# bailuding/rails

Measured on AMD Instinct MI355X. Metric: queries/sec, MoL exact top-k over N items (get_top_k_outputs: score + top-k' + id map + seen-id filter), higher is better.
Workload: dtype f32

## Files before the change

### rails_amd/csrc/mol_score_shell.h

```cpp
#pragma once
#include <hip/hip_runtime.h>
#include <stdlib.h>
#include <type_traits>

#include "mol_kernels.h"
#include "mol_layout.h"

namespace mol {

struct Fp32Unit;
struct Fp32UnitRows;

typedef float f32x16 __attribute__((ext_vector_type(16)));

template <class G, int NW>
__device__ __forceinline__ void stage_weights(const ScoreArgs& p, float* smem) {
  const int lane = threadIdx.x & 63, wave = __builtin_amdgcn_readfirstlane(threadIdx.x >> 6);
  constexpr int kPieces = G::kWpackFloats / 256;
  for (int piece = wave; piece < kPieces; piece += NW)
    __builtin_amdgcn_global_load_lds((const __attribute__((address_space(1))) void*)(p.wpack + piece * 256 + lane * 4),
                                     (__attribute__((address_space(3))) void*)(smem + piece * 256), 16, 0, 0);
  for (int i = kPieces * 256 + threadIdx.x; i < G::kWpackFloats; i += NW * 64) smem[i] = p.wpack[i];
}

template <class U, int PQ, int PX, int DD, int H, int NW, bool INDEXED = false>
__global__ __launch_bounds__(NW * 64, NW / 4) void mol_score_direct_kernel(ScoreArgs p) {
  using G = Geo<PQ, PX, DD, H>;
  MOL_RUN_IF(p.run_if);
  extern __shared__ __attribute__((aligned(16))) float smem[];
  U::template stage<G, NW>(p, smem);
  __syncthreads();

  const int lane = threadIdx.x & 63;
  const int wave = __builtin_amdgcn_readfirstlane(threadIdx.x >> 6);
  const int hi = lane >> 5, x = lane & 31;
  const int inner = p.per_row ? (int)p.n_tiles : p.n_groups;
  const int64_t n_units = p.per_row ? (int64_t)p.B * p.n_tiles : p.n_tiles * p.n_groups;
  const int64_t stride = (int64_t)gridDim.x * NW;
  const int64_t rounds = n_units / stride;
  const int64_t bx = (gridDim.x % 8 == 0) ? (int64_t)(blockIdx.x % 8) * (gridDim.x / 8) + blockIdx.x / 8 : (int64_t)blockIdx.x;
  for (int64_t it = 0; it <= rounds; ++it) {
    const int64_t u = it < rounds ? it * stride + bx * NW + wave
                                  : rounds * stride + (int64_t)wave * gridDim.x + bx;
    if (u >= n_units) break;
    const int64_t outer = u / inner;
    const int innr = (int)(u - outer * inner);
    const int64_t tile = p.per_row ? innr : outer;
    const int row = p.per_row ? (int)outer : -1;
    const int g = p.per_row ? row / G::QT : innr;
    const int64_t tile_addr = p.per_row ? (int64_t)row * p.n_tiles + tile : tile;
    const float4* tEx = reinterpret_cast<const float4*>(p.ipack + tile_addr * (int64_t)G::kTileFloats);
    if constexpr (INDEXED) {
      int col = (int)tile * kTileItems + x;
      col = col < (int)p.n_items ? col : (int)p.n_items - 1;
      int64_t src = p.cand_pos[(int64_t)row * p.n_items + col];
      src = src < 0 ? 0 : (src >= p.index_items ? p.index_items - 1 : src);
      tEx = reinterpret_cast<const float4*>(p.ipack) + (src >> 5) * (int64_t)(G::kTileFloats / 4) + (lane & 32) + (src & 31) - lane;
    }
    const float4* tGi = tEx + G::kTileExFloats / 4;
    const float* eq = p.eqfrag + (int64_t)g * G::kEqGroupFloats;
    f32x16 D1[PX];
    U::template gemm1<G, PX, DD, 1>(D1, eq, tEx, lane);
    U::template queries<G, PX>(D1, p, g, row, tile * kTileItems, smem, tGi, lane, hi, x);
  }
}

template <class UR, int PQ, int PX, int DD, int H, int NW>
__global__ __launch_bounds__(NW * 64, NW / 4) void mol_score_rows_kernel(ScoreArgs p) {
  using G = Geo<PQ, PX, DD, H>;
  MOL_RUN_IF(p.run_if);
  extern __shared__ __attribute__((aligned(16))) float smem[];
  UR::template stage<G, NW>(p, smem);
  __syncthreads();
  constexpr int RP = G::kTileFloats / 4 / kTileItems;
  const int lane = threadIdx.x & 63;
  const int wave = __builtin_amdgcn_readfirstlane(threadIdx.x >> 6);
  const int hi = lane >> 5, x = lane & 31;
  const int64_t n_units = (int64_t)p.B * p.n_tiles;
  const int64_t stride = (int64_t)gridDim.x * NW;
  const int64_t rounds = n_units / stride;
  const int64_t bx = (gridDim.x % 8 == 0) ? (int64_t)(blockIdx.x % 8) * (gridDim.x / 8) + blockIdx.x / 8 : (int64_t)blockIdx.x;
  for (int64_t it = 0; it <= rounds; ++it) {
    const int64_t u = it < rounds ? it * stride + bx * NW + wave : rounds * stride + (int64_t)wave * gridDim.x + bx;
    if (u >= n_units) break;
    const int64_t row64 = u / p.n_tiles;
    const int tile = (int)(u - row64 * p.n_tiles), row = (int)row64;
    int cnt = (int)p.n_items;
    if (p.cand_count) {
      const int c = __builtin_amdgcn_readfirstlane(p.cand_count[row]);
      cnt = c < cnt ? c : cnt;
      if (tile * kTileItems >= cnt) continue;
    }
    int col = tile * kTileItems + x;
    col = col < cnt ? col : cnt - 1;
    int64_t src = p.cand_pos[(int64_t)row * p.n_items + col];
    src = src < 0 ? 0 : (src >= p.index_items ? p.index_items - 1 : src);
    const float4* tEx = reinterpret_cast<const float4*>(p.irows) + src * RP + hi - lane;
    const float4* tGi = tEx + 2 * (G::kTileExFloats / 256);
    const float* eq = p.eqfrag + (int64_t)(row / G::QT) * G::kEqGroupFloats;
    f32x16 D1[PX];
    UR::template gemm1<G, PX, DD, 1>(D1, eq, tEx, lane);
    UR::template queries<G, PX>(D1, p, row / G::QT, row, (int64_t)tile * kTileItems, smem, tGi, lane, hi, x);
  }
}

template <int NW>
__device__ __forceinline__ void dma_floats(const float* __restrict__ src, float* lds, int n_floats, int wave, int lane) {
  for (int piece = wave; piece < n_floats / 256; piece += NW) {
    __builtin_amdgcn_global_load_lds(
        (const __attribute__((address_space(1))) void*)(src + piece * 256 + lane * 4),
        (__attribute__((address_space(3))) void*)(lds + piece * 256), 16, 0, 0);
  }
}

constexpr int kStagedPipe = 0;

template <class U, int PQ, int PX, int DD, int H, int NW>
__global__ __launch_bounds__(NW * 64, NW / 4) void mol_score_staged_kernel(ScoreArgs p) {
  using G = Geo<PQ, PX, DD, H>;
  MOL_RUN_IF(p.run_if);
  static_assert(G::kTileFloats % 256 == 0, "tile must be a whole number of 1 KiB pieces");
  extern __shared__ __attribute__((aligned(16))) float smem[];
  float* tiles = smem + U::template kLdsWeightFloats<G>;
  U::template stage<G, NW>(p, smem);

  const int lane = threadIdx.x & 63;
  const int wave = __builtin_amdgcn_readfirstlane(threadIdx.x >> 6);
  const int hi = lane >> 5, x = lane & 31;
  const int64_t first = blockIdx.x;
  if (first < p.n_tiles) dma_floats<NW>(p.ipack + first * (int64_t)G::kTileFloats, tiles, G::kTileFloats, wave, lane);
  int cur = 0;
  int64_t it = 0;
  for (int64_t tile = first; tile < p.n_tiles; tile += gridDim.x, cur ^= 1, ++it) {
    __syncthreads();
    const int64_t next = tile + gridDim.x;
    if (next < p.n_tiles) dma_floats<NW>(p.ipack + next * (int64_t)G::kTileFloats, tiles + (cur ^ 1) * G::kTileFloats, G::kTileFloats, wave, lane);
    const float4* tEx = reinterpret_cast<const float4*>(tiles + cur * G::kTileFloats);
    const float4* tGi = tEx + G::kTileExFloats / 4;
    for (int g = wave; g < p.n_groups; g += NW) {
      const float* eq = p.eqfrag + (int64_t)g * G::kEqGroupFloats;
      f32x16 D1[PX];
      U::template gemm1<G, PX, DD, kStagedPipe>(D1, eq, tEx, lane);
      U::template queries<G, PX>(D1, p, g, -1, tile * kTileItems, smem, tGi, lane, hi, x);
    }
  }
}

constexpr int kStaged1Pipe = 3;

template <class U, int PQ, int PX, int DD, int H, int NW>
__global__ __launch_bounds__(NW * 64, NW / 4) void mol_score_staged1_kernel(ScoreArgs p) {
  using G = Geo<PQ, PX, DD, H>;
  MOL_RUN_IF(p.run_if);
  static_assert(G::kTileExFloats % 256 == 0 && G::kTileGiFloats % 256 == 0, "1 KiB DMA pieces");
  extern __shared__ __attribute__((aligned(16))) float smem[];
  float* sEx = smem + U::template kLdsWeightFloats<G>;
  float* sGi = sEx + G::kTileExFloats;

  const int lane = threadIdx.x & 63;
  const int wave = __builtin_amdgcn_readfirstlane(threadIdx.x >> 6);
  const int hi = lane >> 5, x = lane & 31;
  const int64_t grid = gridDim.x, b = blockIdx.x;
  const int64_t rounds = p.n_tiles / grid;
  const int64_t left = p.n_tiles - rounds * grid;
  int nsub = 1;
  if (left > 0 && left * 2 <= grid) {
    nsub = (int)(grid / left);
    if (nsub > NW) nsub = NW;
    if (nsub > p.n_groups) nsub = p.n_groups;
  }
  const bool has_left = b < left * nsub;
  const int64_t mine = rounds + (has_left ? 1 : 0);
  if (mine == 0) return;
  U::template stage<G, NW>(p, smem);
  auto tile_of = [&](int64_t i) -> int64_t { return i < rounds ? b + i * grid : rounds * grid + b % left; };

  {
    const float* t0 = p.ipack + tile_of(0) * (int64_t)G::kTileFloats;
    dma_floats<NW>(t0, sEx, G::kTileExFloats, wave, lane);
    dma_floats<NW>(t0 + G::kTileExFloats, sGi, G::kTileGiFloats, wave, lane);
  }
  int cur = 0;
  for (int64_t i = 0; i < mine; ++i, cur ^= 1) {
    const int64_t tile = tile_of(i);
    const bool split_round = i >= rounds && nsub > 1;
    const int off = split_round ? (int)(b / left) : 0, stride = split_round ? nsub : 1;
    const int cnt = (p.n_groups - off + stride - 1) / stride;
    const int n_it = (cnt + NW - 1) / NW;
    __syncthreads();
    const float4* tEx = reinterpret_cast<const float4*>(sEx);
    const float4* tGi = reinterpret_cast<const float4*>(sGi + cur * G::kTileGiFloats);
    for (int it = 0; it < n_it; ++it) {
      const int gi_idx = wave + it * NW;
      const bool has = gi_idx < cnt;
      const int g = off + stride * gi_idx;
      f32x16 D1[PX];
      constexpr int kPipe = (kStaged1Pipe * (PX + 1) > 16 || DD / 8 <= kStaged1Pipe) ? 0 : kStaged1Pipe;
      if (has) U::template gemm1<G, PX, DD, kPipe>(D1, p.eqfrag + (int64_t)g * G::kEqGroupFloats, tEx, lane);
      if (it == n_it - 1) {
        __syncthreads();
        if (i + 1 < mine) {
          const float* tn = p.ipack + tile_of(i + 1) * (int64_t)G::kTileFloats;
          dma_floats<NW>(tn, sEx, G::kTileExFloats, wave, lane);
          dma_floats<NW>(tn + G::kTileExFloats, sGi + (cur ^ 1) * G::kTileGiFloats, G::kTileGiFloats, wave, lane);
        }
      }
      if (has) U::template queries<G, PX>(D1, p, g, -1, tile * kTileItems, smem, tGi, lane, hi, x);
    }
  }
}

inline int score_variant() {
  const char* e = getenv("RAILS_SCORE_VARIANT");
  return e ? atoi(e) : 0;
}

template <class U, int PQ, int PX, int DD, int H, bool STAGED>
static int launch_kernel(const ScoreArgs& a, int n_cu, hipStream_t stream) {
  using G = Geo<PQ, PX, DD, H>;
  constexpr int NW = kScoreWaves;
  constexpr size_t lds = ((size_t)U::template kLdsWeightFloats<G> + (STAGED ? 2 * (size_t)G::kTileFloats : 0)) * sizeof(float);
  if constexpr (lds > 160 * 1024) {
    set_error("staged scoring kernel needs %zu B of LDS", lds);
    return kErrUnsupported;
  } else {
    if (a.dry_run) return kOk;
    int64_t grid;
    if (STAGED) {
      grid = a.n_tiles;
    } else {
      const int64_t n_units = a.per_row ? (int64_t)a.B * a.n_tiles : a.n_tiles * a.n_groups;
      grid = n_units;
    }
    if (grid > (int64_t)n_cu) grid = (int64_t)n_cu;
    if (grid < 1) return kOk;
    auto go = [&](auto kernel) {
      static DynLdsOnce once;
      if (ensure_dyn_lds(once, reinterpret_cast<const void*>(kernel), (int)lds) != kOk) return (int)kErrLaunch;
      hipLaunchKernelGGL(kernel, dim3((unsigned)grid), dim3(NW * 64), lds, stream, a);
      return hipGetLastError() == hipSuccess ? (int)kOk : (int)kErrLaunch;
    };
    if constexpr (STAGED) {
      if (a.cand_pos) { set_error("indexed candidates need the independent-wave shell"); return kErrUnsupported; }
      return go(&mol_score_staged_kernel<U, PQ, PX, DD, H, NW>);
    } else {
      if constexpr (U::kIndexedCandidates) {
        if constexpr (std::is_same_v<U, Fp32Unit>) {
          if (a.cand_pos && a.irows) return go(&mol_score_rows_kernel<Fp32UnitRows, PQ, PX, DD, H, NW>);
        }
        if (a.cand_pos) return go(&mol_score_direct_kernel<U, PQ, PX, DD, H, NW, true>);
      }
      if (a.cand_pos) { set_error("indexed candidates are built for the exact-fp32 kernels only"); return kErrUnsupported; }
      return go(&mol_score_direct_kernel<U, PQ, PX, DD, H, NW>);
    }
  }
}

template <class U, int PQ, int PX, int DD, int H>
static int launch_staged1(const ScoreArgs& a, int n_cu, hipStream_t stream) {
  using G = Geo<PQ, PX, DD, H>;
  constexpr int NW = kScoreWaves;
  constexpr size_t lds = ((size_t)U::template kLdsWeightFloats<G> + (size_t)G::kTileExFloats + 2 * (size_t)G::kTileGiFloats) * sizeof(float);
  if constexpr (lds > 160 * 1024) {
    set_error("single-buffer staged scoring kernel needs %zu B of LDS", lds);
    return kErrUnsupported;
  } else {
    if (a.dry_run) return kOk;
    if (a.n_tiles < 1) return kOk;
    auto go = [&](auto kernel) {
      static DynLdsOnce once;
      if (ensure_dyn_lds(once, reinterpret_cast<const void*>(kernel), (int)lds) != kOk) return (int)kErrLaunch;
      hipLaunchKernelGGL(kernel, dim3((unsigned)n_cu), dim3(NW * 64), lds, stream, a);
      return hipGetLastError() == hipSuccess ? (int)kOk : (int)kErrLaunch;
    };
    return go(&mol_score_staged1_kernel<U, PQ, PX, DD, H, NW>);
  }
}

template <int PQ, int PX, int DD, int H>
inline int choose_variant(const ScoreArgs& a, int n_cu) {
  using G = Geo<PQ, PX, DD, H>;
  constexpr bool staged_fits = ((size_t)G::kWpackFloats + 2 * (size_t)G::kTileFloats) * sizeof(float) <= 160 * 1024;
  constexpr bool staged1_fits = ((size_t)G::kWpackFloats + (size_t)G::kTileExFloats + 2 * (size_t)G::kTileGiFloats) * sizeof(float) <= 160 * 1024;
  int variant = score_variant();
  if (variant == 0) {
    variant = 1;
    if (!a.per_row && a.n_groups >= kScoreWaves) {
      if (staged_fits && a.n_tiles >= 8 * (int64_t)n_cu) variant = 2;
      else if (staged1_fits) variant = 5;
      else if (staged_fits) variant = 2;
    }
  }
  return variant;
}

}
```

Baseline: 11950.

## Defer staged tile prefetch past first GEMM and recompute lane id to cut VGPRs

```diff
diff --git a/rails_amd/csrc/mol_score_shell.h b/rails_amd/csrc/mol_score_shell.h
--- a/rails_amd/csrc/mol_score_shell.h
+++ b/rails_amd/csrc/mol_score_shell.h
@@ -115,6 +115,12 @@
 
 constexpr int kStagedPipe = 0;
 
+__device__ __forceinline__ int lane_now() {
+  int l;
+  asm volatile("v_mbcnt_lo_u32_b32 %0, -1, 0\n\tv_mbcnt_hi_u32_b32 %0, -1, %0" : "=v"(l));
+  return l;
+}
+
 template <class U, int PQ, int PX, int DD, int H, int NW>
 __global__ __launch_bounds__(NW * 64, NW / 4) void mol_score_staged_kernel(ScoreArgs p) {
   using G = Geo<PQ, PX, DD, H>;
@@ -124,25 +130,32 @@
   float* tiles = smem + U::template kLdsWeightFloats<G>;
   U::template stage<G, NW>(p, smem);
 
-  const int lane = threadIdx.x & 63;
   const int wave = __builtin_amdgcn_readfirstlane(threadIdx.x >> 6);
-  const int hi = lane >> 5, x = lane & 31;
-  const int64_t first = blockIdx.x;
-  if (first < p.n_tiles) dma_floats<NW>(p.ipack + first * (int64_t)G::kTileFloats, tiles, G::kTileFloats, wave, lane);
+  const int n_tiles = (int)p.n_tiles, grid = (int)gridDim.x, first = (int)blockIdx.x;
+  if (first < n_tiles) dma_floats<NW>(p.ipack + first * (int64_t)G::kTileFloats, tiles, G::kTileFloats, wave, threadIdx.x & 63);
   int cur = 0;
-  int64_t it = 0;
-  for (int64_t tile = first; tile < p.n_tiles; tile += gridDim.x, cur ^= 1, ++it) {
+  for (int tile = first; tile < n_tiles; tile += grid, cur ^= 1) {
     __syncthreads();
-    const int64_t next = tile + gridDim.x;
-    if (next < p.n_tiles) dma_floats<NW>(p.ipack + next * (int64_t)G::kTileFloats, tiles + (cur ^ 1) * G::kTileFloats, G::kTileFloats, wave, lane);
     const float4* tEx = reinterpret_cast<const float4*>(tiles + cur * G::kTileFloats);
     const float4* tGi = tEx + G::kTileExFloats / 4;
+    bool prefetch = tile + grid < n_tiles;
+    auto issue_prefetch = [&] {
+      __builtin_amdgcn_sched_barrier(0);
+      asm volatile("" ::: "memory");
+      dma_floats<NW>(p.ipack + (tile + grid) * (int64_t)G::kTileFloats, tiles + (cur ^ 1) * G::kTileFloats, G::kTileFloats, wave, lane_now());
+      asm volatile("" ::: "memory");
+      __builtin_amdgcn_sched_barrier(0);
+      prefetch = false;
+    };
     for (int g = wave; g < p.n_groups; g += NW) {
       const float* eq = p.eqfrag + (int64_t)g * G::kEqGroupFloats;
       f32x16 D1[PX];
-      U::template gemm1<G, PX, DD, kStagedPipe>(D1, eq, tEx, lane);
-      U::template queries<G, PX>(D1, p, g, -1, tile * kTileItems, smem, tGi, lane, hi, x);
-    }
+      U::template gemm1<G, PX, DD, kStagedPipe>(D1, eq, tEx, lane_now());
+      if (prefetch) issue_prefetch();
+      const int lane = lane_now();
+      U::template queries<G, PX>(D1, p, g, -1, (int64_t)tile * kTileItems, smem, tGi, lane, lane >> 5, lane & 31);
+    }
+    if (prefetch) issue_prefetch();
   }
 }
 
@@ -159,7 +172,6 @@
 
   const int lane = threadIdx.x & 63;
   const int wave = __builtin_amdgcn_readfirstlane(threadIdx.x >> 6);
-  const int hi = lane >> 5, x = lane & 31;
   const int64_t grid = gridDim.x, b = blockIdx.x;
   const int64_t rounds = p.n_tiles / grid;
   const int64_t left = p.n_tiles - rounds * grid;
@@ -196,16 +208,20 @@
       const int g = off + stride * gi_idx;
       f32x16 D1[PX];
       constexpr int kPipe = (kStaged1Pipe * (PX + 1) > 16 || DD / 8 <= kStaged1Pipe) ? 0 : kStaged1Pipe;
-      if (has) U::template gemm1<G, PX, DD, kPipe>(D1, p.eqfrag + (int64_t)g * G::kEqGroupFloats, tEx, lane);
+      if (has) U::template gemm1<G, PX, DD, kPipe>(D1, p.eqfrag + (int64_t)g * G::kEqGroupFloats, tEx, lane_now());
       if (it == n_it - 1) {
         __syncthreads();
         if (i + 1 < mine) {
           const float* tn = p.ipack + tile_of(i + 1) * (int64_t)G::kTileFloats;
-          dma_floats<NW>(tn, sEx, G::kTileExFloats, wave, lane);
-          dma_floats<NW>(tn + G::kTileExFloats, sGi + (cur ^ 1) * G::kTileGiFloats, G::kTileGiFloats, wave, lane);
+          const int l = lane_now();
+          dma_floats<NW>(tn, sEx, G::kTileExFloats, wave, l);
+          dma_floats<NW>(tn + G::kTileExFloats, sGi + (cur ^ 1) * G::kTileGiFloats, G::kTileGiFloats, wave, l);
         }
       }
-      if (has) U::template queries<G, PX>(D1, p, g, -1, tile * kTileItems, smem, tGi, lane, hi, x);
+      if (has) {
+        const int l = lane_now();
+        U::template queries<G, PX>(D1, p, g, -1, tile * kTileItems, smem, tGi, l, l >> 5, l & 31);
+      }
     }
   }
 }
@@ -242,6 +258,7 @@
     };
     if constexpr (STAGED) {
       if (a.cand_pos) { set_error("indexed candidates need the independent-wave shell"); return kErrUnsupported; }
+      if (a.n_tiles + grid > 0x7fffffff) { set_error("staged scoring kernel counts tiles in 32 bits"); return kErrUnsupported; }
       return go(&mol_score_staged_kernel<U, PQ, PX, DD, H, NW>);
     } else {
       if constexpr (U::kIndexedCandidates) {
```

Result: faster. 12200 (median of 6 runs) (+2.0%).
